# rwdavies/QUILT

Hardware: AMD Instinct MI355X
Metric: samples/sec on 2Mb region, K=50k haps, 1x coverage; dosage r2 vs CPU ref (higher is better)
Workload: dtype f64

## Files before the change

quilt_amd/csrc/gibbs.hip:

```cpp
#include "panel.hpp"

#include <chrono>
#include <functional>

#include <algorithm>
#include <cmath>
#include <cstdlib>
#include <map>
#include <memory>
#include <type_traits>

#include "gibbs_dev.hpp"
#include "gibbs_blocks.hpp"

namespace qa {
int gibbs3_waves(int Ksp, int C, int share);
void launch_gibbs3(const void *gibbs_params, hipStream_t st);
void launch_block_rate3(const void *gibbs_params, hipStream_t st);
void launch_block3(const void *gibbs_params, hipStream_t st);
void launch_resample3(const void *gibbs_params, hipStream_t st);
}

namespace {

// ... 108 lines not shown
    const bool init_iteratively = p.init_iteratively && first_read >= 0;

    if constexpr (SEG) {
        if (p.it_begin > 0) goto sweeps;
    }
    for (int h = 0; h < 3; h++)
        for (int g = t; g < G; g += NT) ch.cv[h][g] = 0.0;
    for (int r = t; r < R; r += NT) ch.Hc[r] = 0;

    {
        Col<NE> one;
#pragma unroll
        for (int i = 0; i < NE; i++) one.v[i] = 1.0;
        for (int h = 0; h < 2; h++)
            for (int g = 0; g < G; g++) ch.st(one, ch.eg[h] + (size_t)g * Ksp);
    }
    chain_sync<NW>();
    if (!init_iteratively) {
        ReadStreams<CH> rs;
        rs.base = -1;
        int r = 0;
        while (r < R) {
            if ((r & 63) == 0 && rs.base != r) rs.load(ch, r, nullptr, 0);
            const int g = rl_i32(rs.wif, r & 63);
            Col<NE> e[2];
#pragma unroll
            for (int i = 0; i < NE; i++) e[0].v[i] = e[1].v[i] = 1.0;
            while (r < R) {
                if ((r & 63) == 0 && rs.base != r) rs.load(ch, r, nullptr, 0);
                if (rl_i32(rs.wif, r & 63) != g) break;
                Col<NE> er;
                {
                    typename CH::ErPre x;
                    ch.ld_pre(x, r);
                    ch.read_emission(er, x, rl_i32(rs.dn, r & 63));
                }
                const int h = rl_i32(rs.H, r & 63) - 1;
#pragma unroll
                for (int i = 0; i < NE; i++) {
                    if (h == 0) e[0].v[i] *= er.v[i];
                    else e[1].v[i] *= er.v[i];
                }
                r++;
            }
            ch.st(e[0], ch.eg[0] + (size_t)g * Ksp);
            ch.st(e[1], ch.eg[1] + (size_t)g * Ksp);
        }
        forward_full_both(ch);
        backward_both<NE, NW, false>(ch);
    } else {
        Col<NE> one;
#pragma unroll
        for (int i = 0; i < NE; i++) one.v[i] = valid[i] ? 1.0 : 0.0;
        for (int h = 0; h < 2; h++) {
            for (int g = 0; g < G; g++) {
                ch.st(one, ch.alpha[h] + (size_t)g * Ksp);
                ch.st(one, ch.beta[h] + (size_t)g * Ksp);
            }
            for (int g = t; g < G; g += NT) ch.cv[h][g] = 1.0;
        }
        chain_sync<NW>();
        for (int h = 0; h < 2; h++) {
            Col<NE> a;
#pragma unroll
            for (int i = 0; i < NE; i++) a.v[i] = valid[i] ? prior * 1.0 : 0.0;
            const double cc = 1 / ch.sum_col(a);
#pragma unroll
            for (int i = 0; i < NE; i++) a.v[i] = a.v[i] * cc;
// ... 87 lines not shown
            double pC[2] = {1, 1};
            if (has) {
                double s[2] = {0, 0};
#pragma unroll
                for (int i = 0; i < NE; i++) {
                    ab[0].v[i] = a[0].v[i] * bt[0].v[i];
                    ab[1].v[i] = a[1].v[i] * bt[1].v[i];
                    s[0] += ab[0].v[i];
                    s[1] += ab[1].v[i];
                }
                ch.template bsum<2>(s);
                pC[0] = s[0]; pC[1] = s[1];
                if constexpr (LEAN) {
#pragma unroll
                    for (int h = 0; h < 2; h++) {
#pragma unroll
                        for (int i = 0; i < NE; i++) s_e[(h * NE + i) * NT + t] = e[h].v[i];
                    }
                }
            }
            int h_rC = 0, h_rA1 = 1;
            bool normal = false, ginit = false, pass = false;
            while (iRead < R) {
                if ((iRead & 63) == 0 && rs.base != iRead) {
                    if (rs.base >= 0) rs.store(ch);
                    rs.load(ch, iRead, runif, it);
                    if (!runif) rs.u = stream_uniform(seed_reads, (uint64_t)R * it + iRead + lane);
                }
                const int jr = iRead & 63;
                if (rl_i32(rs.wif, jr) != g) break;
                const int r = iRead;
                const typename CH::ErPre cur_er = pre_er;
                iRead++;
                ch.ld_pre(pre_er, min(iRead, R - 1), (iRead & 63) ? rl_i32(rs.nent, iRead & 63) : 64);
                if (rl_i32(rs.cat1, jr) != 0) continue;
                Col<NE> er, ri;
                const int dn_r = rl_i32(rs.dn, jr);
                if (dn_r >= 0) {
                    ch.ld(er, ch.eMatRead + (size_t)dn_r * Ksp);
#pragma unroll
                    for (int i = 0; i < NE; i++) ri.v[i] = fast_rcp(er.v[i]);
                } else {
                    ch.expand_with_rcp(er, ri, cur_er);
                }
                if (steady) normal = true;
                else if (r < first_read && it == 0) pass = true;
                else if (first_read <= r && it == 0) { pass = false; ginit = true; }
                else if (r < first_read && it == 1) { pass = false; ginit = true; }
                else { ginit = false; normal = true; }
                double pA1[2] = {pC[0], pC[1]};
                if (normal) {
                    h_rC = rl_i32(rs.H, jr) - 1;
                    h_rA1 = 1 - h_rC;
                    double s[2] = {0, 0};
                    double s2[2] = {0, 0};
                    if (h_rC == 0) {
                        asm volatile("" ::: "memory");
#pragma unroll
                        for (int i = 0; i < NE; i++) {
                            double &u0 = (i & 1) ? s2[0] : s[0], &u1 = (i & 1) ? s2[1] : s[1];
                            u0 += ab[0].v[i] * ri.v[i];
                            u1 += ab[1].v[i] * er.v[i];
                        }
                        asm volatile("; current label 0" : "+v"(s[0]), "+v"(s[1]), "+v"(s2[0]), "+v"(s2[1]));
                    } else {
                        asm volatile("" ::: "memory");
#pragma unroll
                        for (int i = 0; i < NE; i++) {
                            double &u0 = (i & 1) ? s2[0] : s[0], &u1 = (i & 1) ? s2[1] : s[1];
                            u0 += ab[1].v[i] * ri.v[i];
                            u1 += ab[0].v[i] * er.v[i];
                        }
                        asm volatile("; current label 1" : "+v"(s[0]), "+v"(s[1]), "+v"(s2[0]), "+v"(s2[1]));
                    }
                    s[0] += s2[0]; s[1] += s2[1];
                    ch.template bsum<2>(s);
// ... 1178 lines not shown
}

GibbsParams fill_params(const qa::GibbsScratch &S, const qa_panel_t *pn, const qa_rare_common *rc, const qa_gibbs_opts_t *o,
                        const GibbsLaunch &L, const ChunkHost &h, hipStream_t st) {
    const int C = h.C;
    GibbsParams prm{};
    prm.hm = pn->hm.p; prm.B = pn->B.p; prm.sp_off = pn->sp_off.p; prm.sp_k = pn->sp_k.p;
    prm.sp_word = pn->sp_word.p; prm.sigma = S.tm.p; prm.Kp = pn->Kp; prm.G = h.G; prm.T = h.T;
    prm.nMaxDH = pn->nMaxDH; prm.ref_error = pn->ref_error;
    prm.C = C; prm.Ks = h.Ks; prm.Ksp = h.Ksp; prm.NE = h.NE; prm.which = S.which.p;
    prm.read_off = S.read_off.p; prm.read_ptr = S.read_ptr.p; prm.base_off = S.base_off.p;
    prm.u = S.u.p; prm.bq = S.bq.p; prm.wif = S.wif.p; prm.grid_has_read = S.ghr.p;
    prm.pR_tab = S.tabs.p; prm.pA_tab = S.tabs.p + 512;
    prm.Jmax = o->Jmax; prm.inv_maxdiff = 1 / o->maxDifferenceBetweenReads; prm.rescale = o->rescale_eMatRead_t;
    prm.n_its = h.n_its; prm.n_burn_in = o->n_gibbs_burn_in_its; prm.block_its = S.block_its.p;
    prm.n_block = o->perform_block_gibbs ? o->n_block_gibbs_iterations : 0;
    prm.do_shard = o->do_shard_block_gibbs; prm.init_iteratively = o->gibbs_initialize_iteratively;
    prm.disable_read_category_usage = o->disable_read_category_usage;
    prm.class_sum_cutoff = o->class_sum_cutoff;
    prm.nH = h.nH;
    prm.it_begin = 0; prm.it_end = h.n_its;
    prm.ff = o->ff;
    if (o->per_it_out) {
        QA_HIP(hipMemsetAsync(S.per_it.p, 0, sizeof(double) * C * h.n_its * 8, st));
        prm.per_it = S.per_it.p;
    }
    if (L.ff_chain) prm.ff_chain = S.ff_chain.p;
    prm.runif_reads = S.runif_reads.p; prm.first_read = S.first_read.p; prm.runif_shard = S.runif_shard.p;
    prm.seed_reads = L.a.seed_reads ? S.seeds.p : nullptr;
    prm.seed_shard = (L.a.seed_reads && L.a.seed_shard) ? S.seeds.p + C : nullptr;
    prm.eMatRead = S.eMatRead.p; prm.eread_off = S.eread_off.p; prm.is_cat1 = S.is_cat1.p; prm.er_nent = S.er_nent.p;
    prm.er_idx = S.er_idx.p; prm.eridx_off = S.eridx_off.p; prm.er_tab = S.er_tab.p; prm.dense_of = S.dense_of.p;
    prm.er_nt = h.er_nt; prm.er_padb = h.er_padb;
    prm.alpha = S.alpha.p; prm.beta = S.beta.p; prm.eg = S.eg.p; prm.cvec = S.cvec.p;
    prm.H = S.H.p; prm.H_class = S.H_class.p; prm.status = S.status.p;
    prm.hapProbs = S.hap.p; prm.genProbsM = S.gm.p; prm.genProbsF = S.gf.p;
    if (rc) {
        prm.rc_common = rc->common_index.p; prm.rc_rare_ptr = rc->rare_ptr.p; prm.rc_rare_snp = rc->rare_snp.p;
        prm.rc_any = S.rc_any.p; prm.rc_words = h.rc_words; prm.rc_Gc = pn->G;
        if (h.want_pairs) { prm.rc_pairs = S.rc_pairs.p; prm.rc_pair_off = S.rc_pair_off.p; prm.rc_pair_base = S.rc_pair_base.p; }
    }
    return prm;
}

std::vector<int> block_pass_sweeps(const qa_gibbs_opts_t *o, int n_its) {
    std::vector<int> passes;
    if (o->perform_block_gibbs)
        for (int i = 0; i < o->n_block_gibbs_iterations; i++) {
            const int b = o->block_gibbs_iterations[i];
            if (b >= 0 && b < n_its && std::find(passes.begin(), passes.end(), b) == passes.end()) passes.push_back(b);
        }
    std::sort(passes.begin(), passes.end());
    return passes;
}

void block_tables(const qa_gibbs_opts_t *o, const GibbsLaunch &L, const ChunkHost &h, const std::vector<double> &rate2,
                  const std::vector<int32_t> &seg_status, int n_thr, std::vector<int32_t> &h_where, std::vector<int32_t> &h_tab,
                  std::vector<int32_t> &h_n) {
    const int C = h.C, G = h.G;
    const int32_t *read_off = L.a.read_off;
    h_where.assign((size_t)C * G, -1); h_tab.assign((size_t)C * 4 * G, 0); h_n.assign(C, 0);
    qa::parallel_for((size_t)C, n_thr, [&](size_t c) {
        const int R = read_off[c + 1] - read_off[c];
        if (seg_status[c] != 0) return;
        if (R < 1 || (h.nH == 2 && G < 3)) {
            if (h.nH == 2) { h_n[c] = 1; h_tab[c * 4 * G + G] = G - 1; h_where[c * G + G - 1] = 0; }
// ... 660 lines not shown
```

quilt_amd/csrc/gibbs3.hip:

```cpp
#include "gibbs_dev.hpp"

#include <type_traits>

namespace {

template <int NE, int NW, bool LEAN = false>
__global__ __launch_bounds__(64 * NW) __attribute__((amdgpu_waves_per_eu(LEAN ? 2 : NW))) void k_gibbs3(GibbsParams p) {
    __shared__ double s_red[2 * NW * 4];
    __shared__ double s_e[LEAN ? 3 * NE * 64 * NW : 1];
    const int c = blockIdx.x, t = threadIdx.x;
    using CH = Chain<NE, NW>;
    CH ch(p, c, t, s_red);
    constexpr int NT = CH::NT;
    constexpr int NH = 3;
    const int G = ch.G, Ksp = ch.Ksp, R = ch.R, Ks = ch.Ks;
    const double prior = ch.prior;
    bool (&valid)[NE] = ch.valid;
    const double *runif = p.seed_reads ? nullptr : p.runif_reads + (size_t)p.read_off[c] * p.n_its;
    const uint64_t seed_reads = p.seed_reads ? p.seed_reads[c] : 0;
    const int first_read = p.first_read[c];
    const bool init_iteratively = p.init_iteratively && first_read >= 0;
    const double one_over_K = 1 / (double)Ks;

    auto sum3 = [&](const Col<NE> (&x)[NH], double (&s)[NH]) {
#pragma unroll
        for (int h = 0; h < NH; h++) {
            s[h] = 0;
#pragma unroll
            for (int i = 0; i < NE; i++) s[h] += x[h].v[i];
        }
        ch.template bsum<NH>(s);
    };
// ... 71 lines not shown
                else ch.st(b[h], ch.beta[h] + (size_t)g * Ksp);
            }
#pragma unroll
            for (int h = 0; h < NH; h++) e[h] = en[h];
        }
        chain_sync<NW>();
    };

    auto build_forward = [&](bool store_alpha) {
        ReadStreams<CH> rs;
        rs.load(ch, 0, nullptr, 0);
        typename CH::ErPre pre{};
        if (R > 0) ch.ld_pre(pre, 0);
        int r = 0;
        Col<NE> a[NH];
        GridStreams3<CH> gs;
        for (int g = 0; g < G; g++) {
            if ((g & 63) == 0) {
                if (g) gs.store_c(ch);
                gs.load_fwd(ch, g);
            }
            const int jg = g & 63;
            Col<NE> e[NH];
#pragma unroll
            for (int h = 0; h < NH; h++)
#pragma unroll
                for (int i = 0; i < NE; i++) e[h].v[i] = 1.0;
            bool any = false;
            while (r < R) {
                if (r >= rs.base + 64) rs.load(ch, r, nullptr, 0);
                const int j = r - rs.base;
                if (rl_i32(rs.wif, j) != g) break;
                const typename CH::ErPre x = pre;
                ch.ld_pre(pre, min(r + 1, R - 1));
                Col<NE> er;
                ch.read_emission(er, x, rl_i32(rs.dn, j));
                const int hh = rl_i32(rs.H, j) - 1;
#pragma unroll
                for (int h = 0; h < NH; h++)
                    if (hh == h) {
#pragma unroll
                        for (int i = 0; i < NE; i++) e[h].v[i] *= er.v[i];
                    }
                any = true;
                r++;
            }
            if (any) {
#pragma unroll
                for (int h = 0; h < NH; h++) ch.st(e[h], ch.eg[h] + (size_t)g * Ksp);
            }
            const double s0 = rl_f64(gs.t0, jg), s1 = rl_f64(gs.t1, jg);
#pragma unroll
            for (int h = 0; h < NH; h++) {
#pragma unroll
                for (int i = 0; i < NE; i++) {
                    if (g == 0) a[h].v[i] = valid[i] ? prior * e[h].v[i] : 0.0;
                    else a[h].v[i] = valid[i] ? e[h].v[i] * (s0 * a[h].v[i] + s1 * prior) : 0.0;
                }
            }
            double sm[NH], cc[NH];
            sum3(a, sm);
#pragma unroll
            for (int h = 0; h < NH; h++) {
                cc[h] = 1 / sm[h];
#pragma unroll
                for (int i = 0; i < NE; i++) a[h].v[i] = a[h].v[i] * cc[h];
                if (store_alpha) ch.st(a[h], ch.alpha[h] + (size_t)g * Ksp);
            }
            gs.set_c(ch.lane, jg, cc[0], cc[1], cc[2]);
// ... 119 lines not shown
                for (int h = 0; h < NH; h++) ch.ldm(bt[h], ch.beta[h] + gn);
            }
            bool grid_started = false, changed = false;
            int moved = 0;
            double pC[3] = {1, 1, 1};
            bool normal = false, ginit = false, pass = false;
            while (iRead < R) {
                if (iRead >= rs.base + 64) {
                    if (rs_dirty) { rs.store(ch); rs_dirty = false; }
                    rs_load(iRead);
                }
                const int j = iRead - rs.base;
                if (rl_i32(rs.wif, j) != g) break;
                const int r = iRead;
                iRead++;
                if (!init_iteratively) normal = true;
                else if (r < first_read && it == 0) pass = true;
                else if (first_read <= r && it == 0) { pass = false; ginit = true; }
                else if (r < first_read && it == 1) { pass = false; ginit = true; }
                else { ginit = false; normal = true; }
                if (!grid_started) {
                    sum3(ab, pC);
                    grid_started = true;
                    if constexpr (LEAN) {
#pragma unroll
                        for (int h = 0; h < NH; h++)
#pragma unroll
                            for (int i = 0; i < NE; i++) s_e[(h * NE + i) * NT + t] = e[h].v[i];
                    }
                }
                Col<NE> er, rer;
                {
                    const typename CH::ErPre x = pre;
                    ch.ld_pre(pre, min(r + 1, R - 1));
                    const int dn_r = rl_i32(rs.dn, j);
                    if (dn_r >= 0) {
                        ch.ld(er, ch.eMatRead + (size_t)dn_r * Ksp);
#pragma unroll
                        for (int i = 0; i < NE; i++) rer.v[i] = fast_rcp(er.v[i]);
                    } else {
                        ch.expand_with_rcp(er, rer, x);
                    }
                }
                int h_rC = 0, h_rA1 = 1, h_rN = 0;
                double pA1[3] = {pC[0], pC[1], pC[2]}, pA2[3] = {pC[0], pC[1], pC[2]};
                double x3[3];
                const double chance = rl_f64(rs.u, j);
                auto draw = [&](auto HC) {
                    constexpr int hc = decltype(HC)::value, a1 = hc == 0 ? 1 : 0, a2 = hc == 2 ? 1 : 2;
                    const double prod_pC = (pC[0] * pC[1] * pC[2]) * pp[hc];
                    const double prod_pA1 = (pA1[0] * pA1[1] * pA1[2]) * pp[a1];
                    const double prod_pA2 = (pA2[0] * pA2[1] * pA2[2]) * pp[a2];
                    const double denom = prod_pC + prod_pA1 + prod_pA2;
                    const double rden = fast_rcp(denom);
                    x3[hc] = prod_pC * rden; x3[a1] = prod_pA1 * rden; x3[a2] = prod_pA2 * rden;
                    const double cs0 = x3[0], cs1 = x3[1] + cs0, cs2 = x3[2] + cs1;
                    h_rN = 0;
                    if (chance < cs2) h_rN = 2;
                    if (chance < cs1) h_rN = 1;
                    if (chance < cs0) h_rN = 0;
                };
                auto normal_read = [&](auto HC) {
                    constexpr int hc = decltype(HC)::value, a1 = hc == 0 ? 1 : 0, a2 = hc == 2 ? 1 : 2;
                    h_rA1 = a1;
                    if (rl_i32(rs.cat1, j) == 0) {
                        double s[3] = {0, 0, 0};
#pragma unroll
                        for (int i = 0; i < NE; i++) {
                            s[0] += ab[0].v[i] * (hc == 0 ? rer.v[i] : er.v[i]);
                            s[1] += ab[1].v[i] * (hc == 1 ? rer.v[i] : er.v[i]);
                            s[2] += ab[2].v[i] * (hc == 2 ? rer.v[i] : er.v[i]);
                        }
                        ch.template bsum<3>(s);
                        pA1[hc] = s[hc]; pA1[a1] = s[a1];
// ... 199 lines not shown
    return perm[2];
}

__device__ inline double log_p_H_class2(const int (&n)[6], double ff) {
    return 0 + n[0] * log(0.5) + n[1] * log(0.5 - ff * 0.5) + n[2] * log(ff * 0.5) + n[3] * log(1 - ff * 0.5) +
           n[4] * log(1 * 0.5 + ff * 0.5) + n[5] * log(1 * 0.5);
}

template <int NE, int NW>
__global__ __launch_bounds__(64 * NW) void k_block3(GibbsParams p) {
    __shared__ double s_red[2 * NW * 4];
    const int c = blockIdx.x, t = threadIdx.x;
    using CH = Chain<NE, NW>;
    CH ch(p, c, t, s_red);
    constexpr int NT = CH::NT;
    constexpr int NH = 3;
    constexpr int RR[6][3] = {{1, 2, 3}, {1, 3, 2}, {2, 1, 3}, {2, 3, 1}, {3, 1, 2}, {3, 2, 1}};
    constexpr int RX[6][3] = {{1, 2, 3}, {1, 3, 2}, {2, 1, 3}, {3, 1, 2}, {2, 3, 1}, {3, 2, 1}};
    const int G = ch.G, Ksp = ch.Ksp, R = ch.R, Ks = ch.Ks;
    const double prior = ch.prior, one_over_K = 1 / (double)Ks;
    const double ff = p.ff_chain ? rl_f64(p.ff_chain[c], 0) : p.ff;
    bool (&valid)[NE] = ch.valid;
    if (__builtin_amdgcn_readfirstlane(p.status[c]) != 0) return;
    auto uni_d = [](const double *q) { return rl_f64(*q, 0); };
    auto uni_i = [](int v) { return __builtin_amdgcn_readfirstlane(v); };
    const int32_t *where = p.blk_where + (size_t)c * G;
    const int32_t *tab = p.blk_tab + (size_t)c * 4 * G;
    const int n_blocks = uni_i(p.blk_n[c]);
    const double *ru = p.seed_shard ? nullptr : p.runif_shard + ((size_t)p.read_off[c] * p.blk_n_pass + (size_t)p.blk_pass * R) * 2;
    const uint64_t seed = p.seed_shard ? p.seed_shard[c] : 0;
    auto u_block = [&](int i) { return ru ? ru[i] : stream_uniform(seed, (uint64_t)p.blk_pass * 2 * R + i); };
    auto u_draw = [&](int r) { return ru ? ru[R + r] : stream_uniform(seed, (uint64_t)p.blk_pass * 2 * R + R + r); };
    const bool foreign = NW == 2 && p.er_nt == 64;
    int rb_base = -1, rb_wif = 0, rb_H = 0, rb_dn = 0;
    auto rb_get = [&](int r) {
        if (rb_base < 0 || r < rb_base || r >= rb_base + 64) {
            rb_base = r & ~63;
            const int q = rb_base + ch.lane;
            const bool ok = q < R;
            rb_wif = ok ? ch.wif[q] : -1;
            rb_H = ok ? ch.H[q] : 1;
            rb_dn = ok ? ch.dense_of[q] : -1;
        }
        return r - rb_base;
    };
    auto wif_of = [&](int r) { const int j = rb_get(r); return rl_i32(rb_wif, j); };
    auto H_of = [&](int r) { const int j = rb_get(r); return rl_i32(rb_H, j); };
    auto emission_of = [&](Col<NE> &er, int r) {
        const int dn = rl_i32(rb_dn, rb_get(r));
        if (dn >= 0) { ch.ld(er, ch.eMatRead + (size_t)dn * Ksp); return; }
        if (!foreign) {
            typename CH::ErPre x;
            ch.ld_pre(x, r);
            ch.expand(er, x);
            return;
        }
        struct __attribute__((packed, aligned(4))) U3 { uint32_t a, b, c; };
        const U3 q = *reinterpret_cast<const U3 *>(ch.eridx + ((size_t)r * 64 + ch.lane) * 12);
        const uint32_t w4[4] = {q.a, q.b, q.c, 0u};
        const double tv = ch.ertab[(size_t)r * 64 + ch.lane];
        const int lo = __double2loint(tv), hi = __double2hiint(tv);
#pragma unroll
        for (int i = 0; i < NE; i++) {
            uint32_t code = 0;
#pragma unroll
            for (int b = 0; b < 12; b++)
                if (b == ch.wave + 2 * i) code = (w4[b >> 2] >> ((b & 3) * 8)) & 0xffu;
            const int src = (int)code << 2;
            er.v[i] = __hiloint2double(__builtin_amdgcn_ds_bpermute(src, hi), __builtin_amdgcn_ds_bpermute(src, lo));
        }
    };
    auto sum3 = [&](const Col<NE> (&x)[NH], double (&s)[NH]) {
#pragma unroll
        for (int h = 0; h < NH; h++) {
            s[h] = 0;
#pragma unroll
            for (int i = 0; i < NE; i++) s[h] += x[h].v[i];
        }
        ch.template bsum<NH>(s);
    };

    constexpr int EM[6][3] = {{0, 1, 2}, {0, 2, 1}, {1, 0, 2}, {2, 0, 1}, {1, 2, 0}, {2, 1, 0}};
    Col<NE> aS[3][3];
    double inside[3][3];
    double logC_before[3] = {0, 0, 0}, logC_after[3];
    {
        double s[3] = {0, 0, 0};
        for (int g = t; g < G; g += NT)
#pragma unroll
            for (int h = 0; h < 3; h++) s[h] += log(ch.cv[h][g]);
        ch.template bsum<3>(s);
#pragma unroll
        for (int h = 0; h < 3; h++) logC_after[h] = s[h];
    }
#pragma unroll
    for (int h = 0; h < 3; h++)
#pragma unroll
        for (int i = 0; i < 3; i++) inside[h][i] = 0;
    bool ever_changed = false;

// ... 319 lines not shown
```

quilt_amd/csrc/gibbs_dev.hpp:

```cpp
#pragma once

#include "panel.hpp"

#include <cstdint>

namespace {

struct GibbsParams {
    const uint8_t *hm;
    const int32_t *B;
    const int32_t *sp_off;
    const int32_t *sp_k;
    const uint32_t *sp_word;
    const double *sigma;
    int Kp, G, T, nMaxDH;
    double ref_error;
    int C;
    int Ks, Ksp, NE;
    const int32_t *which;
    const int32_t *read_off;
    const int32_t *read_ptr;
    const int32_t *base_off;
    const int32_t *u;
    const int32_t *bq;
    const int32_t *wif;
    const uint8_t *grid_has_read;
    const double *pR_tab, *pA_tab;
    int Jmax;
    double inv_maxdiff;
    int rescale;
    int n_its, n_burn_in;
    const int32_t *block_its;
    int n_block;
    int do_shard;
    int init_iteratively;
    int nH;
    int disable_read_category_usage;
    double class_sum_cutoff;
    const double *runif_reads;
    const int32_t *first_read;
    const double *runif_shard;
    const uint64_t *seed_reads, *seed_shard;
    double *eMatRead;
    const size_t *eread_off;
    uint8_t *er_idx;
    const size_t *eridx_off;
    double *er_tab;
    const int32_t *dense_of;
    int er_nt, er_padb;
    uint8_t *is_cat1;
    uint8_t *er_nent;
    double *alpha, *beta, *eg;
    double *cvec;
    int32_t *H;
    int32_t *H_class;
    int32_t *status;
    double *hapProbs, *genProbsM, *genProbsF;
    const int32_t *rc_common;
    const int64_t *rc_rare_ptr;
    const int32_t *rc_rare_snp;
    const uint32_t *rc_any;
    int rc_words, rc_Gc;
    const int32_t *rc_pair_off;
    const size_t *rc_pair_base;
    const uint16_t *rc_pairs;
    int it_begin, it_end;
    int rebuild;
    int lean3;
    const int32_t *blk_where;
    const int32_t *blk_tab;
    const int32_t *blk_n;
    double *blk_rate2;
    int blk_pass, blk_n_pass;
    int defer_resample;
    double ff;
    const double *ff_chain;
    double *per_it;
};

__device__ __forceinline__ bool rare_has_alt(const GibbsParams &p, int hap, int snp) {
    int64_t lo = p.rc_rare_ptr[hap], hi = p.rc_rare_ptr[hap + 1];
    while (lo < hi) {
// ... 65 lines not shown
#pragma unroll
    for (int o = 32; o > 0; o >>= 1) v = fmax(v, __shfl_xor(v, o, 64));
    return v;
}

__device__ __forceinline__ double stream_uniform(uint64_t seed, uint64_t i) {
    uint64_t z = seed + (i + 1) * 0x9E3779B97F4A7C15ull;
    z = (z ^ (z >> 30)) * 0xBF58476D1CE4E5B9ull;
    z = (z ^ (z >> 27)) * 0x94D049BB133111EBull;
    z = z ^ (z >> 31);
    return (double)(z >> 11) * (1.0 / 9007199254740992.0);
}

__device__ __forceinline__ uint32_t panel_word(const GibbsParams &p, int g, int k, int code) {
    if (code > 0) return (uint32_t)p.B[(size_t)g * p.nMaxDH + (code - 1)];
    int lo = p.sp_off[g], hi = p.sp_off[g + 1] - 1;
    while (lo < hi) {
        int mid = (lo + hi) >> 1;
        if (p.sp_k[mid] < k) lo = mid + 1; else hi = mid;
    }
    return p.sp_word[lo];
}

__device__ __forceinline__ double rl_f64(double v, int j) {
    const int lo = __builtin_amdgcn_readlane(__double2loint(v), j);
    const int hi = __builtin_amdgcn_readlane(__double2hiint(v), j);
    return __hiloint2double(hi, lo);
}
__device__ __forceinline__ int rl_i32(int v, int j) { return __builtin_amdgcn_readlane(v, j); }

constexpr int kReadsPerWave = 32;
constexpr int kMaxPatternBits = 5;
constexpr int padb_of(int ne) { return ne <= 4 ? 4 : ne <= 8 ? 8 : ne <= 12 ? 12 : 16; }

template <int NEALL, int NW>
__global__ __launch_bounds__(64) void k_ematread(GibbsParams p) {
    constexpr int NE = NEALL / NW, PADB = padb_of(NE), NT = 64 * NW;
    const int c = blockIdx.y, lane = threadIdx.x;
    const int R = p.read_off[c + 1] - p.read_off[c];
    const int r0 = blockIdx.x * kReadsPerWave;
    if (r0 >= R) return;
    const int32_t *rp = p.read_ptr + p.read_off[c] + c;
    const int32_t *u = p.u + p.base_off[c], *bq = p.bq + p.base_off[c];
    const int32_t *which = p.which + (size_t)c * p.Ks;
    int kk[NEALL];
#pragma unroll
    for (int i = 0; i < NEALL; i++) {
        const int k = lane + 64 * i;
        kk[i] = (k < p.Ks) ? which[k] : -1;
    }
    int g_prev = -1;
    uint32_t w[NEALL];
    const double e1 = 1 - p.ref_error, e0 = p.ref_error;
    const int nblk = min(kReadsPerWave, R - r0);
    static_assert(kReadsPerWave < 64, "lane l holds the offset of read r0 + l, lane nblk the block's end");
    const int my_s = (lane <= nblk) ? rp[r0 + lane] : 0;
    const int my_dense = (lane < nblk) ? p.dense_of[p.read_off[c] + r0 + lane] : -1;
    const int b_end = rl_i32(my_s, nblk);
    int chunk0 = rl_i32(my_s, 0), c_u = 0, c_b = 0;
    double c_R = 0, c_A = 0;
    auto load_chunk = [&](int base) {
        chunk0 = base;
        const int idx = base + lane;
        const bool ok = idx < b_end;
        c_u = ok ? u[idx] : 0;
        c_b = ok ? bq[idx] : 0;
// ... 67 lines not shown
                pat[i] |= bit << min(n_inf, 7);
            }
            tv *= ((lane >> min(n_inf, 31)) & 1) ? f1 : f0;
            n_inf++;
        }
        bool degenerate = false;
        double d1 = 1.0;
        if (p.rescale) {
            double x = 0;
#pragma unroll
            for (int i = 0; i < NEALL; i++) if (kk[i] >= 0 && v[i] > x) x = v[i];
            x = wmax(x);
            d1 = 1 / x;
            degenerate = isinf(x) || x == 0 || isinf(d1);
            if (degenerate) {
#pragma unroll
                for (int i = 0; i < NEALL; i++) v[i] = 1;
                tv = 1;
            } else {
#pragma unroll
                for (int i = 0; i < NEALL; i++) {
                    v[i] *= d1;
                    if (v[i] < p.inv_maxdiff) v[i] = p.inv_maxdiff;
                }
                tv *= d1;
                if (tv < p.inv_maxdiff) tv = p.inv_maxdiff;
            }
        }
        const double thresh = 1 - 1e-12;
        bool below = false;
#pragma unroll
        for (int i = 0; i < NEALL; i++) if (kk[i] >= 0 && v[i] < thresh) below = true;
        const bool any_below = __any(below);
        if (lane == 0) {
            p.is_cat1[p.read_off[c] + r] = (any_below || p.disable_read_category_usage) ? 0 : 1;
            p.er_nent[p.read_off[c] + r] = (uint8_t)(n_inf <= kMaxPatternBits ? (1 << n_inf) : 64);
        }
        if (dense >= 0) {
            double *out = p.eMatRead + p.eread_off[c] + (size_t)dense * p.Ksp;
#pragma unroll
            for (int i = 0; i < NEALL; i++) out[lane + 64 * i] = (kk[i] >= 0) ? v[i] : 1.0;
        } else {
            p.er_tab[(size_t)(p.read_off[c] + r) * 64 + lane] = (lane < (1 << n_inf) && lane != 63) ? tv : 1.0;
            uint8_t *ix = p.er_idx + p.eridx_off[c] + (size_t)r * NT * PADB;
#pragma unroll
            for (int wv = 0; wv < NW; wv++) {
                uint32_t pk[PADB / 4];
#pragma unroll
                for (int q = 0; q < PADB / 4; q++) pk[q] = 0;
#pragma unroll
                for (int i = 0; i < NE; i++) {
                    const int j = wv + NW * i;
                    const uint32_t code = (kk[j] >= 0 && !degenerate) ? pat[j] : 63u;
                    pk[i >> 2] |= code << ((i & 3) * 8);
                }
                uint32_t *dst = reinterpret_cast<uint32_t *>(ix + (size_t)(lane + 64 * wv) * PADB);
#pragma unroll
                for (int q = 0; q < PADB / 4; q++) dst[q] = pk[q];
            }
        }
    }
}

template <int NE>
struct Col {
    double v[NE];
};

__device__ __forceinline__ __amdgpu_buffer_rsrc_t buf_rsrc(const void *base, uint32_t bytes) {
    return __builtin_amdgcn_make_buffer_rsrc(const_cast<void *>(base), 0, (int)bytes, 0x00020000);
}
__device__ __forceinline__ double buf_ld_f64(__amdgpu_buffer_rsrc_t r, uint32_t byte_off) {
    return __builtin_bit_cast(double, __builtin_amdgcn_raw_buffer_load_b64(r, (int)byte_off, 0, 0));
}
__device__ __forceinline__ void buf_st_f64(__amdgpu_buffer_rsrc_t r, uint32_t byte_off, double v) {
    __builtin_amdgcn_raw_buffer_store_b64(__builtin_bit_cast(__attribute__((__vector_size__(2 * sizeof(unsigned int)))) unsigned int, v), r,
                                          (int)byte_off, 0, 0);
}

template <int NE>
__device__ __forceinline__ void load_col(Col<NE> &c, const double *src, int t, int NT) {
#pragma unroll
    for (int i = 0; i < NE; i++) c.v[i] = src[t + NT * i];
}
template <int NE>
__device__ __forceinline__ void store_col(const Col<NE> &c, double *dst, int t, int NT) {
#pragma unroll
    for (int i = 0; i < NE; i++) dst[t + NT * i] = c.v[i];
}

__device__ __forceinline__ double fast_rcp(double e) {
    double r = __builtin_amdgcn_rcp(e);
    r = __builtin_fma(__builtin_fma(-e, r, 1.0), r, r);
    r = __builtin_fma(__builtin_fma(-e, r, 1.0), r, r);
    return r;
}

template <int NE, int NW>
struct Chain {
    static constexpr int NT = 64 * NW;
    const GibbsParams &p;
    int c, t, lane, wave, R, G, Ks, Ksp;
    double *alpha[3], *beta[3], *eg[3], *cv[3];
    const double *eMatRead;
    const uint8_t *eridx;
    const double *ertab;
    const int32_t *dense_of;
    const int32_t *wif;
    const uint8_t *ghr, *cat1, *nent;
    int32_t *H, *Hc;
    double prior;
    bool valid[NE];
    double *red;
    int par;

    __device__ Chain(const GibbsParams &p_, int c_, int t_, double *red_)
        : p(p_), c(c_), t(t_), lane(t_ & 63), wave(t_ >> 6), red(red_), par(0) {
        G = p.G; Ks = p.Ks; Ksp = p.Ksp;
        R = p.read_off[c + 1] - p.read_off[c];
        const size_t mat = (size_t)G * Ksp;
        for (int h = 0; h < 3; h++) {
            const size_t at = ((size_t)c * p.nH + min(h, p.nH - 1)) * mat;
            alpha[h] = p.alpha + at;
            beta[h] = p.beta + at;
            eg[h] = p.eg + at;
        }
        for (int h = 0; h < 3; h++) cv[h] = p.cvec + ((size_t)c * 3 + h) * G;
        eMatRead = p.eMatRead + p.eread_off[c];
        eridx = p.er_idx + p.eridx_off[c];
        ertab = p.er_tab + (size_t)p.read_off[c] * 64;
        dense_of = p.dense_of + p.read_off[c];
        wif = p.wif + p.read_off[c];
        cat1 = p.is_cat1 + p.read_off[c];
        nent = p.er_nent + p.read_off[c];
        ghr = p.grid_has_read + (size_t)c * G;
        H = p.H + p.read_off[c];
        Hc = p.H_class + p.read_off[c];
        prior = 1.0 / Ks;
#pragma unroll
        for (int i = 0; i < NE; i++) valid[i] = (i < NE - 1) ? true : (t + NT * i) < Ks;
    }
    static constexpr int PADB = padb_of(NE);
    struct ErPre {
        uint32_t w[PADB / 4];
        double tv;
    };
    __device__ __forceinline__ void ld_pre(ErPre &x, int r, int nent = 64) const {
        const uint32_t *src = reinterpret_cast<const uint32_t *>(eridx + ((size_t)r * NT + t) * PADB);
        if constexpr (PADB == 16) {
            const uint4 q = *reinterpret_cast<const uint4 *>(src);
            x.w[0] = q.x; x.w[1] = q.y; x.w[2] = q.z; x.w[3] = q.w;
        } else if constexpr (PADB == 12) {
            struct __attribute__((packed, aligned(4))) U3 { uint32_t a, b, c; };
            const U3 q = *reinterpret_cast<const U3 *>(src);
            x.w[0] = q.a; x.w[1] = q.b; x.w[2] = q.c;
        } else if constexpr (PADB == 8) {
            const uint2 q = *reinterpret_cast<const uint2 *>(src);
            x.w[0] = q.x; x.w[1] = q.y;
        } else {
            x.w[0] = *src;
        }
        const double tv = buf_ld_f64(buf_rsrc(ertab + (size_t)r * 64, (uint32_t)nent * 8), (uint32_t)lane * 8);
        x.tv = lane == 63 ? 1.0 : tv;
    }
    __device__ __forceinline__ void expand(Col<NE> &er, const ErPre &x) const {
        const int lo = __double2loint(x.tv), hi = __double2hiint(x.tv);
#pragma unroll
        for (int i = 0; i < NE; i++) {
            const int src = (int)((x.w[i >> 2] >> ((i & 3) * 8)) & 0xffu) << 2;
            er.v[i] = __hiloint2double(__builtin_amdgcn_ds_bpermute(src, hi), __builtin_amdgcn_ds_bpermute(src, lo));
        }
    }
    __device__ __forceinline__ void expand_with_rcp(Col<NE> &er, Col<NE> &ri, const ErPre &x) const {
        const double tvi = fast_rcp(x.tv);
        const int lo = __double2loint(x.tv), hi = __double2hiint(x.tv);
        const int ilo = __double2loint(tvi), ihi = __double2hiint(tvi);
#pragma unroll
        for (int i = 0; i < NE; i++) {
            const int src = (int)((x.w[i >> 2] >> ((i & 3) * 8)) & 0xffu) << 2;
            er.v[i] = __hiloint2double(__builtin_amdgcn_ds_bpermute(src, hi), __builtin_amdgcn_ds_bpermute(src, lo));
            ri.v[i] = __hiloint2double(__builtin_amdgcn_ds_bpermute(src, ihi), __builtin_amdgcn_ds_bpermute(src, ilo));
        }
    }
    __device__ __forceinline__ void read_emission(Col<NE> &er, const ErPre &x, int dn) const {
        if (dn >= 0) ld(er, eMatRead + (size_t)dn * Ksp);
        else expand(er, x);
    }

    __device__ __forceinline__ double tm0(int g) const { return p.sigma[g]; }
    __device__ __forceinline__ double tm1(int g) const { return p.sigma[p.G - 1 + g]; }

    template <int N>
    __device__ __forceinline__ void bsum(double (&x)[N]) {
        if constexpr (N == 1) x[0] = wsum(x[0]);
        if constexpr (N == 2) wsum2(x[0], x[1]);
        if constexpr (N == 3) wsum3(x[0], x[1], x[2]);
        if constexpr (N == 4) wsum4(x[0], x[1], x[2], x[3]);
        static_assert(N >= 1 && N <= 4, "bsum handles 1..4 values");
        if (NW == 1) return;
        double *buf = red + (size_t)par * NW * 4;
        if (lane == 0) {
#pragma unroll
            for (int q = 0; q < N; q++) buf[wave * 4 + q] = x[q];
        }
        asm volatile("s_waitcnt lgkmcnt(0)" ::: "memory");
        __builtin_amdgcn_s_barrier();
        asm volatile("" ::: "memory");
#pragma unroll
        for (int q = 0; q < N; q++) {
            double s = 0;
#pragma unroll
            for (int w = 0; w < NW; w++) s += buf[w * 4 + q];
            x[q] = s;
        }
        par ^= 1;
    }
    __device__ __forceinline__ double bsum1(double v) {
        double x[1] = {v};
        bsum<1>(x);
// ... 130 lines not shown
```

Before: 36.96.

## Pack read-emission indices into narrow bitfields with planar layout

Reads with few distinct emission patterns now have their per-haplotype pattern codes stored as narrow bitfields in a single 32-bit word instead of one byte per entry. The index array also switches from interleaved to planar layout, so the loader fetches only the planes it needs, and it skips the fetch entirely for dense or category-1 reads. The intent is to cut global memory traffic for the read emission indices in the Gibbs kernels, at the cost of branchy decode logic and a per-read nent lookup. An environment variable can disable the packing.

```diff
diff --git a/quilt_amd/csrc/gibbs.hip b/quilt_amd/csrc/gibbs.hip
--- a/quilt_amd/csrc/gibbs.hip
+++ b/quilt_amd/csrc/gibbs.hip
@@ -164,8 +164,9 @@
                 Col<NE> er;
                 {
                     typename CH::ErPre x;
-                    ch.ld_pre(x, r);
-                    ch.read_emission(er, x, rl_i32(rs.dn, r & 63));
+                    const int dn_r = rl_i32(rs.dn, r & 63), nent_r = rl_i32(rs.nent, r & 63);
+                    ch.ld_pre_as(x, r, nent_r, dn_r, false);
+                    ch.read_emission(er, x, dn_r, nent_r);
                 }
                 const int h = rl_i32(rs.H, r & 63) - 1;
 #pragma unroll
@@ -319,7 +320,8 @@
                 const int r = iRead;
                 const typename CH::ErPre cur_er = pre_er;
                 iRead++;
-                ch.ld_pre(pre_er, min(iRead, R - 1), (iRead & 63) ? rl_i32(rs.nent, iRead & 63) : 64);
+                ch.ld_pre_as(pre_er, min(iRead, R - 1), rl_i32(rs.nent, iRead & 63), rl_i32(rs.dn, iRead & 63),
+                             rl_i32(rs.cat1, iRead & 63) != 0, (iRead & 63) != 0);
                 if (rl_i32(rs.cat1, jr) != 0) continue;
                 Col<NE> er, ri;
                 const int dn_r = rl_i32(rs.dn, jr);
@@ -328,7 +330,7 @@
 #pragma unroll
                     for (int i = 0; i < NE; i++) ri.v[i] = fast_rcp(er.v[i]);
                 } else {
-                    ch.expand_with_rcp(er, ri, cur_er);
+                    ch.expand_with_rcp(er, ri, cur_er, rl_i32(rs.nent, jr));
                 }
                 if (steady) normal = true;
                 else if (r < first_read && it == 0) pass = true;
@@ -1573,6 +1575,8 @@
     prm.eMatRead = S.eMatRead.p; prm.eread_off = S.eread_off.p; prm.is_cat1 = S.is_cat1.p; prm.er_nent = S.er_nent.p;
     prm.er_idx = S.er_idx.p; prm.eridx_off = S.eridx_off.p; prm.er_tab = S.er_tab.p; prm.dense_of = S.dense_of.p;
     prm.er_nt = h.er_nt; prm.er_padb = h.er_padb;
+    const char *forms_env = getenv("QA_GIBBS_PACK_FORMS");
+    prm.pack_forms = (forms_env && atoi(forms_env) == 0) ? 0 : 1;
     prm.alpha = S.alpha.p; prm.beta = S.beta.p; prm.eg = S.eg.p; prm.cvec = S.cvec.p;
     prm.H = S.H.p; prm.H_class = S.H_class.p; prm.status = S.status.p;
     prm.hapProbs = S.hap.p; prm.genProbsM = S.gm.p; prm.genProbsF = S.gf.p;
diff --git a/quilt_amd/csrc/gibbs3.hip b/quilt_amd/csrc/gibbs3.hip
--- a/quilt_amd/csrc/gibbs3.hip
+++ b/quilt_amd/csrc/gibbs3.hip
@@ -1,3 +1,4 @@
+#define QA_PACK_DECODE_SELECT
 #include "gibbs_dev.hpp"
 
 #include <type_traits>
@@ -135,9 +136,9 @@
                 const int j = r - rs.base;
                 if (rl_i32(rs.wif, j) != g) break;
                 const typename CH::ErPre x = pre;
-                ch.ld_pre(pre, min(r + 1, R - 1));
+                ch.ld_pre_as(pre, min(r + 1, R - 1), rl_i32(rs.nent, (j + 1) & 63), rl_i32(rs.dn, (j + 1) & 63), false, j < 63);
                 Col<NE> er;
-                ch.read_emission(er, x, rl_i32(rs.dn, j));
+                ch.read_emission(er, x, rl_i32(rs.dn, j), rl_i32(rs.nent, j));
                 const int hh = rl_i32(rs.H, j) - 1;
 #pragma unroll
                 for (int h = 0; h < NH; h++)
@@ -323,14 +324,14 @@
                 Col<NE> er, rer;
                 {
                     const typename CH::ErPre x = pre;
-                    ch.ld_pre(pre, min(r + 1, R - 1));
+                    ch.ld_pre_as(pre, min(r + 1, R - 1), rl_i32(rs.nent, (j + 1) & 63), rl_i32(rs.dn, (j + 1) & 63), false, j < 63);
                     const int dn_r = rl_i32(rs.dn, j);
                     if (dn_r >= 0) {
                         ch.ld(er, ch.eMatRead + (size_t)dn_r * Ksp);
 #pragma unroll
                         for (int i = 0; i < NE; i++) rer.v[i] = fast_rcp(er.v[i]);
                     } else {
-                        ch.expand_with_rcp(er, rer, x);
+                        ch.expand_with_rcp(er, rer, x, rl_i32(rs.nent, j));
                     }
                 }
                 int h_rC = 0, h_rA1 = 1, h_rN = 0;
@@ -596,7 +597,7 @@
     auto u_block = [&](int i) { return ru ? ru[i] : stream_uniform(seed, (uint64_t)p.blk_pass * 2 * R + i); };
     auto u_draw = [&](int r) { return ru ? ru[R + r] : stream_uniform(seed, (uint64_t)p.blk_pass * 2 * R + R + r); };
     const bool foreign = NW == 2 && p.er_nt == 64;
-    int rb_base = -1, rb_wif = 0, rb_H = 0, rb_dn = 0;
+    int rb_base = -1, rb_wif = 0, rb_H = 0, rb_dn = 0, rb_nent = 0;
     auto rb_get = [&](int r) {
         if (rb_base < 0 || r < rb_base || r >= rb_base + 64) {
             rb_base = r & ~63;
@@ -605,6 +606,7 @@
             rb_wif = ok ? ch.wif[q] : -1;
             rb_H = ok ? ch.H[q] : 1;
             rb_dn = ok ? ch.dense_of[q] : -1;
+            rb_nent = ok ? ch.nent[q] : 64;
         }
         return r - rb_base;
     };
@@ -613,23 +615,29 @@
     auto emission_of = [&](Col<NE> &er, int r) {
         const int dn = rl_i32(rb_dn, rb_get(r));
         if (dn >= 0) { ch.ld(er, ch.eMatRead + (size_t)dn * Ksp); return; }
+        const int nent = rl_i32(rb_nent, rb_get(r));
         if (!foreign) {
             typename CH::ErPre x;
-            ch.ld_pre(x, r);
-            ch.expand(er, x);
+            ch.ld_pre_as(x, r, nent, dn, false);
+            ch.expand(er, x, nent);
             return;
         }
-        struct __attribute__((packed, aligned(4))) U3 { uint32_t a, b, c; };
-        const U3 q = *reinterpret_cast<const U3 *>(ch.eridx + ((size_t)r * 64 + ch.lane) * 12);
-        const uint32_t w4[4] = {q.a, q.b, q.c, 0u};
+        const bool narrow = pack_is_narrow<10>(p, nent);
+        uint32_t w3[3];
+        ld_planes<12, 64>(w3, ch.eridx, r, ch.lane, narrow ? 1 : 3);
+        const uint32_t w4[4] = {w3[0], w3[1], w3[2], 0u};
         const double tv = ch.ertab[(size_t)r * 64 + ch.lane];
         const int lo = __double2loint(tv), hi = __double2hiint(tv);
 #pragma unroll
         for (int i = 0; i < NE; i++) {
             uint32_t code = 0;
-#pragma unroll
-            for (int b = 0; b < 12; b++)
-                if (b == ch.wave + 2 * i) code = (w4[b >> 2] >> ((b & 3) * 8)) & 0xffu;
+            if (narrow) {
+                code = (i == NE - 1 && !valid[NE - 1]) ? 63u : (w4[0] >> (3 * (ch.wave + 2 * i))) & 7u;
+            } else {
+#pragma unroll
+                for (int b = 0; b < 12; b++)
+                    if (b == ch.wave + 2 * i) code = (w4[b >> 2] >> ((b & 3) * 8)) & 0xffu;
+            }
             const int src = (int)code << 2;
             er.v[i] = __hiloint2double(__builtin_amdgcn_ds_bpermute(src, hi), __builtin_amdgcn_ds_bpermute(src, lo));
         }
diff --git a/quilt_amd/csrc/gibbs_dev.hpp b/quilt_amd/csrc/gibbs_dev.hpp
--- a/quilt_amd/csrc/gibbs_dev.hpp
+++ b/quilt_amd/csrc/gibbs_dev.hpp
@@ -48,6 +48,7 @@
     double *er_tab;
     const int32_t *dense_of;
     int er_nt, er_padb;
+    int pack_forms;
     uint8_t *is_cat1;
     uint8_t *er_nent;
     double *alpha, *beta, *eg;
@@ -179,6 +180,12 @@
 constexpr int kReadsPerWave = 32;
 constexpr int kMaxPatternBits = 5;
 constexpr int padb_of(int ne) { return ne <= 4 ? 4 : ne <= 8 ? 8 : ne <= 12 ? 12 : 16; }
+constexpr int narrow_bits_of(int ne) { return ne <= 4 ? 0 : 32 / ne; }
+template <int NE>
+__device__ __forceinline__ bool pack_is_narrow(const GibbsParams &p, int nent) {
+    constexpr int FB = narrow_bits_of(NE);
+    return FB > 0 && p.pack_forms != 0 && nent <= (1 << FB);
+}
 
 template <int NEALL, int NW>
 __global__ __launch_bounds__(64) void k_ematread(GibbsParams p) {
@@ -312,9 +319,10 @@
 #pragma unroll
         for (int i = 0; i < NEALL; i++) if (kk[i] >= 0 && v[i] < thresh) below = true;
         const bool any_below = __any(below);
+        const int nent = n_inf <= kMaxPatternBits ? (1 << n_inf) : 64;
         if (lane == 0) {
             p.is_cat1[p.read_off[c] + r] = (any_below || p.disable_read_category_usage) ? 0 : 1;
-            p.er_nent[p.read_off[c] + r] = (uint8_t)(n_inf <= kMaxPatternBits ? (1 << n_inf) : 64);
+            p.er_nent[p.read_off[c] + r] = (uint8_t)nent;
         }
         if (dense >= 0) {
             double *out = p.eMatRead + p.eread_off[c] + (size_t)dense * p.Ksp;
@@ -322,9 +330,22 @@
             for (int i = 0; i < NEALL; i++) out[lane + 64 * i] = (kk[i] >= 0) ? v[i] : 1.0;
         } else {
             p.er_tab[(size_t)(p.read_off[c] + r) * 64 + lane] = (lane < (1 << n_inf) && lane != 63) ? tv : 1.0;
-            uint8_t *ix = p.er_idx + p.eridx_off[c] + (size_t)r * NT * PADB;
+            uint32_t *ix = reinterpret_cast<uint32_t *>(p.er_idx + p.eridx_off[c] + (size_t)r * NT * PADB);
+            constexpr int FB = narrow_bits_of(NE);
+            const bool narrow = pack_is_narrow<NE>(p, nent);
 #pragma unroll
             for (int wv = 0; wv < NW; wv++) {
+                uint32_t *dst = ix + lane + 64 * wv;
+                if (narrow) {
+                    uint32_t pk = 0;
+#pragma unroll
+                    for (int i = 0; i < NE; i++) {
+                        const int j = wv + NW * i;
+                        pk |= (kk[j] >= 0 ? pat[j] & ((1u << FB) - 1) : 0u) << ((i * FB) & 31);
+                    }
+                    dst[0] = pk;
+                    continue;
+                }
                 uint32_t pk[PADB / 4];
 #pragma unroll
                 for (int q = 0; q < PADB / 4; q++) pk[q] = 0;
@@ -334,9 +355,8 @@
                     const uint32_t code = (kk[j] >= 0 && !degenerate) ? pat[j] : 63u;
                     pk[i >> 2] |= code << ((i & 3) * 8);
                 }
-                uint32_t *dst = reinterpret_cast<uint32_t *>(ix + (size_t)(lane + 64 * wv) * PADB);
-#pragma unroll
-                for (int q = 0; q < PADB / 4; q++) dst[q] = pk[q];
+#pragma unroll
+                for (int q = 0; q < PADB / 4; q++) dst[q * NT] = pk[q];
             }
         }
     }
@@ -356,6 +376,13 @@
 __device__ __forceinline__ void buf_st_f64(__amdgpu_buffer_rsrc_t r, uint32_t byte_off, double v) {
     __builtin_amdgcn_raw_buffer_store_b64(__builtin_bit_cast(__attribute__((__vector_size__(2 * sizeof(unsigned int)))) unsigned int, v), r,
                                           (int)byte_off, 0, 0);
+}
+
+template <int PADB_, int NT_>
+__device__ __forceinline__ void ld_planes(uint32_t (&w)[PADB_ / 4], const uint8_t *eridx, int r, int t, int planes) {
+    const __amdgpu_buffer_rsrc_t slot = buf_rsrc(eridx + (size_t)r * NT_ * PADB_, (uint32_t)planes * NT_ * 4);
+#pragma unroll
+    for (int j = 0; j < PADB_ / 4; j++) w[j] = (uint32_t)__builtin_amdgcn_raw_buffer_load_b32(slot, (j * NT_ + t) * 4, 0, 0);
 }
 
 template <int NE>
@@ -419,52 +446,132 @@
         prior = 1.0 / Ks;
 #pragma unroll
         for (int i = 0; i < NE; i++) valid[i] = (i < NE - 1) ? true : (t + NT * i) < Ks;
-    }
+#ifdef QA_DBG_PACK_READ0
+        dbg_r = 0;
+        while (dbg_r < R - 1 && __builtin_amdgcn_readfirstlane(dense_of[dbg_r]) >= 0) dbg_r++;
+#endif
+    }
+#ifdef QA_DBG_PACK_READ0
+    int dbg_r;
+#endif
     static constexpr int PADB = padb_of(NE);
     struct ErPre {
         uint32_t w[PADB / 4];
         double tv;
     };
-    __device__ __forceinline__ void ld_pre(ErPre &x, int r, int nent = 64) const {
-        const uint32_t *src = reinterpret_cast<const uint32_t *>(eridx + ((size_t)r * NT + t) * PADB);
-        if constexpr (PADB == 16) {
-            const uint4 q = *reinterpret_cast<const uint4 *>(src);
-            x.w[0] = q.x; x.w[1] = q.y; x.w[2] = q.z; x.w[3] = q.w;
-        } else if constexpr (PADB == 12) {
-            struct __attribute__((packed, aligned(4))) U3 { uint32_t a, b, c; };
-            const U3 q = *reinterpret_cast<const U3 *>(src);
-            x.w[0] = q.a; x.w[1] = q.b; x.w[2] = q.c;
-        } else if constexpr (PADB == 8) {
-            const uint2 q = *reinterpret_cast<const uint2 *>(src);
-            x.w[0] = q.x; x.w[1] = q.y;
-        } else {
-            x.w[0] = *src;
-        }
+    static constexpr int NPL = PADB / 4;
+    static constexpr int FB = narrow_bits_of(NE);
+    __device__ __forceinline__ void ld_pre(ErPre &x, int r, int planes = NPL, int nent = 64) const {
+#ifdef QA_DBG_PACK_READ0
+        r = dbg_r; planes = NPL; nent = 64;
+        asm volatile("" : "+s"(r));
+#endif
+        ld_planes<PADB, NT>(x.w, eridx, r, t, planes);
         const double tv = buf_ld_f64(buf_rsrc(ertab + (size_t)r * 64, (uint32_t)nent * 8), (uint32_t)lane * 8);
         x.tv = lane == 63 ? 1.0 : tv;
     }
-    __device__ __forceinline__ void expand(Col<NE> &er, const ErPre &x) const {
+    __device__ __forceinline__ void ld_pre_as(ErPre &x, int r, int nent, int dn, bool skipped, bool known = true) const {
+        const bool none = known && p.pack_forms != 0 && (dn >= 0 || skipped);
+        const bool narrow = known && pack_is_narrow<NE>(p, nent);
+        ld_pre(x, r, none ? 0 : (narrow ? 1 : NPL), none ? 0 : (known ? nent : 64));
+    }
+    template <bool NARROW>
+    __device__ __forceinline__ int code4(const ErPre &x, int i) const {
+        if constexpr (NARROW) {
+            const uint32_t f = (x.w[0] >> ((i * FB) & 31)) & ((1u << FB) - 1);
+            return (int)((i == NE - 1 && !valid[NE - 1]) ? 63u : f) << 2;
+        } else {
+            return (int)((x.w[i >> 2] >> ((i & 3) * 8)) & 0xffu) << 2;
+        }
+    }
+    struct Merged {
+        uint32_t w[NPL];
+        bool narrow;
+    };
+    __device__ __forceinline__ Merged merge(const ErPre &x, bool narrow) const {
+        Merged m;
+        m.narrow = narrow;
+#pragma unroll
+        for (int q = 0; q < NPL; q++) m.w[q] = (q > 0 && narrow) ? x.w[0] : x.w[q];
+        return m;
+    }
+    __device__ __forceinline__ int code4(const Merged &m, int i) const {
+        const uint32_t sh = m.narrow ? (uint32_t)((i * FB) & 31) : (uint32_t)((i & 3) * 8), mask = m.narrow ? (1u << FB) - 1 : 0xffu;
+        const uint32_t f = (m.w[i >> 2] >> sh) & mask;
+        return (int)((i == NE - 1 && m.narrow && !valid[NE - 1]) ? 63u : f) << 2;
+    }
+    template <bool NARROW>
+    __device__ __forceinline__ void expand_as(Col<NE> &er, const ErPre &x) const {
         const int lo = __double2loint(x.tv), hi = __double2hiint(x.tv);
 #pragma unroll
         for (int i = 0; i < NE; i++) {
-            const int src = (int)((x.w[i >> 2] >> ((i & 3) * 8)) & 0xffu) << 2;
+            const int src = code4<NARROW>(x, i);
             er.v[i] = __hiloint2double(__builtin_amdgcn_ds_bpermute(src, hi), __builtin_amdgcn_ds_bpermute(src, lo));
         }
     }
-    __device__ __forceinline__ void expand_with_rcp(Col<NE> &er, Col<NE> &ri, const ErPre &x) const {
-        const double tvi = fast_rcp(x.tv);
+    __device__ __forceinline__ void expand(Col<NE> &er, const ErPre &x, int nent) const {
+        if constexpr (FB == 0) {
+            expand_as<false>(er, x);
+#ifdef QA_PACK_DECODE_SELECT
+        } else if (true) {
+            const Merged m = merge(x, pack_is_narrow<NE>(p, nent));
+            const int lo = __double2loint(x.tv), hi = __double2hiint(x.tv);
+#pragma unroll
+            for (int i = 0; i < NE; i++) {
+                const int src = code4(m, i);
+                er.v[i] = __hiloint2double(__builtin_amdgcn_ds_bpermute(src, hi), __builtin_amdgcn_ds_bpermute(src, lo));
+            }
+#endif
+        } else if (pack_is_narrow<NE>(p, nent)) {
+            asm volatile("" ::: "memory");
+            expand_as<true>(er, x);
+            asm volatile("; narrow form" : "+v"(er.v[0]));
+        } else {
+            asm volatile("" ::: "memory");
+            expand_as<false>(er, x);
+            asm volatile("; byte form" : "+v"(er.v[0]));
+        }
+    }
+    template <bool NARROW>
+    __device__ __forceinline__ void expand_with_rcp_as(Col<NE> &er, Col<NE> &ri, const ErPre &x, double tvi) const {
         const int lo = __double2loint(x.tv), hi = __double2hiint(x.tv);
         const int ilo = __double2loint(tvi), ihi = __double2hiint(tvi);
 #pragma unroll
         for (int i = 0; i < NE; i++) {
-            const int src = (int)((x.w[i >> 2] >> ((i & 3) * 8)) & 0xffu) << 2;
+            const int src = code4<NARROW>(x, i);
             er.v[i] = __hiloint2double(__builtin_amdgcn_ds_bpermute(src, hi), __builtin_amdgcn_ds_bpermute(src, lo));
             ri.v[i] = __hiloint2double(__builtin_amdgcn_ds_bpermute(src, ihi), __builtin_amdgcn_ds_bpermute(src, ilo));
         }
     }
-    __device__ __forceinline__ void read_emission(Col<NE> &er, const ErPre &x, int dn) const {
+    __device__ __forceinline__ void expand_with_rcp(Col<NE> &er, Col<NE> &ri, const ErPre &x, int nent) const {
+        const double tvi = fast_rcp(x.tv);
+        if constexpr (FB == 0) {
+            expand_with_rcp_as<false>(er, ri, x, tvi);
+#ifdef QA_PACK_DECODE_SELECT
+        } else if (true) {
+            const Merged m = merge(x, pack_is_narrow<NE>(p, nent));
+            const int lo = __double2loint(x.tv), hi = __double2hiint(x.tv);
+            const int ilo = __double2loint(tvi), ihi = __double2hiint(tvi);
+#pragma unroll
+            for (int i = 0; i < NE; i++) {
+                const int src = code4(m, i);
+                er.v[i] = __hiloint2double(__builtin_amdgcn_ds_bpermute(src, hi), __builtin_amdgcn_ds_bpermute(src, lo));
+                ri.v[i] = __hiloint2double(__builtin_amdgcn_ds_bpermute(src, ihi), __builtin_amdgcn_ds_bpermute(src, ilo));
+            }
+#endif
+        } else if (pack_is_narrow<NE>(p, nent)) {
+            asm volatile("" ::: "memory");
+            expand_with_rcp_as<true>(er, ri, x, tvi);
+            asm volatile("; narrow form" : "+v"(er.v[0]), "+v"(ri.v[0]));
+        } else {
+            asm volatile("" ::: "memory");
+            expand_with_rcp_as<false>(er, ri, x, tvi);
+            asm volatile("; byte form" : "+v"(er.v[0]), "+v"(ri.v[0]));
+        }
+    }
+    __device__ __forceinline__ void read_emission(Col<NE> &er, const ErPre &x, int dn, int nent) const {
         if (dn >= 0) ld(er, eMatRead + (size_t)dn * Ksp);
-        else expand(er, x);
+        else expand(er, x, nent);
     }
 
     __device__ __forceinline__ double tm0(int g) const { return p.sigma[g]; }
```

After: 36.64. About the same (-0.9%).
